# Ray0089/geometric-aware-dense-matching

Measured on AMD Instinct MI355X. Metric: rgbd_crops_per_sec_geomatch_fwd, higher is better.
Workload: dtype bf16x3/f32acc

## Files before the change

geometric_aware_dense_matching_amd/csrc/gdm_lfa.hip:

```cpp
#include "gdm_common.h"
#include <math.h>
#include <stdlib.h>

namespace {

constexpr int LK = 16;

struct LfaArgs {
    const float* xyz;
    const int32_t* idx;
    const float* feat;
    const float* w1t;
    const float* s1;
    const float* b1;
    const float* w2t;
    const float* s2;
    const float* b2;
    const float* wft;
    const float* wmt;
    const float* sm;
    const float* bm;
    float* out;
    int n, OUT;
    float slope;
};

__device__ __forceinline__ float lrelu(float v, float slope) { return v > 0.f ? v : v * slope; }



__device__ __forceinline__ float quadrow_max(float v)
{
    v = fmaxf(v, __shfl_xor(v, 16));
    v = fmaxf(v, __shfl_xor(v, 32));
    return v;
}
__device__ __forceinline__ float quadrow_sum(float v, int kq)
{
    float o = __shfl_xor(v, 16);
    v = (kq & 1) ? o + v : v + o;
    o = __shfl_xor(v, 32);
    v = (kq & 2) ? o + v : v + o;
    return v;
}

template <int ROWS, int KD, int NRT, int NPT, int WR, int WP>
__device__ __forceinline__ void lfa_tiles(const float* __restrict__ wt, const float* src, int src_pstride, int rt0, int pt0, int l16, int kq,
                                          gdm_f32x4 (&acc)[NRT][NPT])
{
#pragma unroll
    for (int i = 0; i < NRT; ++i)
#pragma unroll
        for (int j = 0; j < NPT; ++j)
#pragma unroll
            for (int r = 0; r < 4; ++r) acc[i][j][r] = 0.f;
    const float* wl = wt + (long)kq * ROWS + rt0 * 16 + l16;
    const float* sl = src + (long)pt0 * src_pstride + kq * LK + l16;
    constexpr int G = 4;
    static_assert(KD % (4 * G) == 0, "KD in whole groups");
    float an[G][NRT];
#pragma unroll
    for (int g = 0; g < G; ++g)
#pragma unroll
        for (int i = 0; i < NRT; ++i) an[g][i] = wl[(long)(4 * g) * ROWS + i * WR * 16];
    for (int jj = 0; jj < KD; jj += 4 * G) {
        float ac[G][NRT], bv[G][NPT];
#pragma unroll
        for (int g = 0; g < G; ++g)
#pragma unroll
            for (int i = 0; i < NRT; ++i) ac[g][i] = an[g][i];
        if (jj + 4 * G < KD) {
#pragma unroll
            for (int g = 0; g < G; ++g)
#pragma unroll
                for (int i = 0; i < NRT; ++i) an[g][i] = wl[(long)(jj + 4 * G + 4 * g) * ROWS + i * WR * 16];
        }
#pragma unroll
        for (int g = 0; g < G; ++g)
#pragma unroll
            for (int j = 0; j < NPT; ++j) bv[g][j] = sl[(jj + 4 * g) * LK + j * WP * src_pstride];
#pragma unroll
        for (int g = 0; g < G; ++g)
#pragma unroll
            for (int i = 0; i < NRT; ++i)
#pragma unroll
                for (int j = 0; j < NPT; ++j) acc[i][j] = __builtin_amdgcn_mfma_f32_16x16x4f32(bv[g][j], ac[g][i], acc[i][j], 0, 0, 0);
    }
}

template <int D, int PP>
__global__ __launch_bounds__(256) void lfa_stage_mfma_kernel(const LfaArgs a)
{
    constexpr int H = D / 2;
    constexpr int P = (256 / D) * PP;
    __shared__ __attribute__((aligned(16))) float fcat[P][D][LK];
    __shared__ __attribute__((aligned(16))) float fx1[P][H][LK];
    __shared__ float pe[P][10][LK];
    __shared__ int nidx[P][LK];
    __shared__ float aggv[P][D];

    const int tid = threadIdx.x;
    const int slot = tid / D, c = tid - slot * D;
    const int lane = tid & 63, wave = tid >> 6, l16 = lane & 15, kq = lane >> 4;
    const int b = blockIdx.y;
    const int n = a.n;
    const float slope = a.slope;
    int pidx[PP];
    bool live[PP];
#pragma unroll
    for (int pp = 0; pp < PP; ++pp) {
        const int raw = (int)blockIdx.x * P + slot * PP + pp;
        live[pp] = raw < n;
        pidx[pp] = min(raw, n - 1);
    }

    if (c < LK) {
#pragma unroll
        for (int pp = 0; pp < PP; ++pp) {
            const int p = slot * PP + pp, i = pidx[pp];
            int jn = a.idx[((long)b * n + i) * LK + c];
            jn = min(max(jn, 0), n - 1);
            const float* pi = a.xyz + ((long)b * n + i) * 3;
            const float* pj = a.xyz + ((long)b * n + jn) * 3;
            const float ax = pi[0], ay = pi[1], az = pi[2];
            const float bx = pj[0], by = pj[1], bz = pj[2];
            const float rx = __fsub_rn(ax, bx), ry = __fsub_rn(ay, by), rz = __fsub_rn(az, bz);
            float s = __fmul_rn(rx, rx);
            s = __fadd_rn(s, __fmul_rn(ry, ry));
            s = __fadd_rn(s, __fmul_rn(rz, rz));
            pe[p][0][c] = __fsqrt_rn(s);
            pe[p][1][c] = rx; pe[p][2][c] = ry; pe[p][3][c] = rz;
            pe[p][4][c] = ax; pe[p][5][c] = ay; pe[p][6][c] = az;
            pe[p][7][c] = bx; pe[p][8][c] = by; pe[p][9][c] = bz;
            nidx[p][c] = jn;
        }
    }
    __syncthreads();

    {
        const int j = c % H, kb = (c / H) * 8;
        float w[10];
#pragma unroll
        for (int q = 0; q < 10; ++q) w[q] = a.w1t[q * H + j];
        const float sc = a.s1[j], sh = a.b1[j];
        const float* frow = a.feat + ((long)b * H + j) * n;
#pragma unroll
        for (int pp = 0; pp < PP; ++pp) {
            const int p = slot * PP + pp;
#pragma unroll
            for (int kk = 0; kk < 8; ++kk) {
                const int k = kb + kk;
                float v = 0.f;
#pragma unroll
                for (int q = 0; q < 10; ++q) v = fmaf(w[q], pe[p][q][k], v);
                v = lrelu(fmaf(v, sc, sh), slope);
                if (a.w2t) fx1[p][j][k] = v;
                else fcat[p][H + j][k] = v;
                fcat[p][j][k] = frow[nidx[p][k]];
            }
        }
    }
    __syncthreads();

    if (a.w2t) {
        constexpr int RT = H / 16, WR = RT < 4 ? RT : 4, WP = 4 / WR, NRT = RT / WR, NPT = P / WP;
        static_assert(RT >= 1 && NRT * WR == RT && NPT * WP == P, "mlp2 tiling");
        const int wr = wave % WR, wp = wave / WR;
        gdm_f32x4 acc[NRT][NPT];
        lfa_tiles<H, H, NRT, NPT, WR, WP>(a.w2t, &fx1[0][0][0], H * LK, wr, wp, l16, kq, acc);
#pragma unroll
        for (int i = 0; i < NRT; ++i) {
            const int ch = (wr + WR * i) * 16 + l16;
            const float sc = a.s2[ch], sh = a.b2[ch];
#pragma unroll
            for (int j = 0; j < NPT; ++j) {
                float4 o;
                o.x = lrelu(fmaf(acc[i][j][0], sc, sh), slope); o.y = lrelu(fmaf(acc[i][j][1], sc, sh), slope);
                o.z = lrelu(fmaf(acc[i][j][2], sc, sh), slope); o.w = lrelu(fmaf(acc[i][j][3], sc, sh), slope);
                *reinterpret_cast<float4*>(&fcat[wp + WP * j][H + ch][4 * kq]) = o;
            }
        }
        __syncthreads();
    }

    {
        constexpr int RT = D / 16, WR = RT < 4 ? RT : 4, WP = 4 / WR, NRT = RT / WR, NPT = P / WP;
        static_assert(NRT * WR == RT && NPT * WP == P, "attention tiling");
        const int wr = wave % WR, wp = wave / WR;
        gdm_f32x4 acc[NRT][NPT];
        lfa_tiles<D, D, NRT, NPT, WR, WP>(a.wft, &fcat[0][0][0], D * LK, wr, wp, l16, kq, acc);
#pragma unroll
        for (int i = 0; i < NRT; ++i) {
            const int ch = (wr + WR * i) * 16 + l16;
#pragma unroll
            for (int j = 0; j < NPT; ++j) {
                const int p = wp + WP * j;
                const gdm_f32x4 t = acc[i][j];
                const float mx = quadrow_max(fmaxf(fmaxf(t[0], t[1]), fmaxf(t[2], t[3])));
                const float e0 = __expf(t[0] - mx), e1 = __expf(t[1] - mx), e2 = __expf(t[2] - mx), e3 = __expf(t[3] - mx);
                const float den = quadrow_sum((e0 + e1) + (e2 + e3), kq);
                const float4 f = *reinterpret_cast<const float4*>(&fcat[p][ch][4 * kq]);
                const float rden = 1.0f / den;
                const float num = quadrow_sum((f.x * (e0 * rden) + f.y * (e1 * rden)) + (f.z * (e2 * rden) + f.w * (e3 * rden)), kq);
                if (kq == 0) aggv[p][ch] = num;
            }
        }
    }
    __syncthreads();

    const int OUT = a.OUT;
    if (c < OUT) {
        float o[PP];
#pragma unroll
        for (int pp = 0; pp < PP; ++pp) o[pp] = 0.f;
#pragma unroll 8
        for (int jj = 0; jj < D; ++jj) {
            const float w = a.wmt[jj * OUT + c];
#pragma unroll
            for (int pp = 0; pp < PP; ++pp) o[pp] = fmaf(w, aggv[slot * PP + pp][jj], o[pp]);
        }
        const float sm = a.sm[c], bm = a.bm[c];
#pragma unroll
        for (int pp = 0; pp < PP; ++pp)
            if (live[pp]) a.out[((long)b * OUT + c) * n + pidx[pp]] = lrelu(fmaf(o[pp], sm, bm), slope);
    }
}

}

extern "C" int gdm_lfa_stage_hip(const float* xyz, const int32_t* idx, const float* feat, const float* w1t, const float* s1, const float* b1,
                                 const float* w2t, const float* s2, const float* b2, const float* wft, const float* wmt, const float* sm,
                                 const float* bm, int B, int n, int K, int D, int OUT, float slope, float* out, void* stream)
{
    GDM_CHECK_ARG(xyz && idx && feat && w1t && s1 && b1 && wft && wmt && sm && bm && out, "gdm_lfa_stage_hip: NULL pointer");
    GDM_CHECK_ARG(!w2t || (s2 && b2), "gdm_lfa_stage_hip: w2t without s2/b2");
    GDM_CHECK_ARG(K == LK, "gdm_lfa_stage_hip: K=%d, only K=16 is built", K);
    GDM_CHECK_ARG(D == 32 || D == 64 || D == 128 || D == 256, "gdm_lfa_stage_hip: D=%d not in {32,64,128,256}", D);
    GDM_CHECK_ARG(OUT >= 1 && OUT <= D, "gdm_lfa_stage_hip: OUT=%d must be in [1, D=%d]", OUT, D);
    GDM_CHECK_ARG(B >= 1 && B <= 65535 && n >= 1, "gdm_lfa_stage_hip: bad shape");
    LfaArgs a{xyz, idx, feat, w1t, s1, b1, w2t, s2, b2, wft, wmt, sm, bm, out, n, OUT, slope};
    hipStream_t s = (hipStream_t)stream;
    const int pp = D <= 64 ? 1 : 2;
    const int P = (256 / D) * pp;
    dim3 g(gdm_cdiv(n, P), B);
    if (D == 32) hipLaunchKernelGGL((lfa_stage_mfma_kernel<32, 1>), g, dim3(256), 0, s, a);
    else if (D == 64) hipLaunchKernelGGL((lfa_stage_mfma_kernel<64, 1>), g, dim3(256), 0, s, a);
    else if (D == 128) hipLaunchKernelGGL((lfa_stage_mfma_kernel<128, 2>), g, dim3(256), 0, s, a);
    else hipLaunchKernelGGL((lfa_stage_mfma_kernel<256, 2>), g, dim3(256), 0, s, a);
    return gdm_launch_status("lfa_stage_mfma_kernel");
}
```

geometric_aware_dense_matching_amd/csrc/gdm_pointwise.hip:

```cpp
#include "gdm_common.h"
#include <stdlib.h>

namespace {

constexpr int PT = 64, XS = 68;
constexpr int MAXSEG = 4;

struct PwSegDev {
    const float* x;
    const int32_t* idx;
    int C, n_src;
};

struct PwArgs {
    PwSegDev seg[MAXSEG];
    int nseg;
    const float* wt;
    long wks, wcs;
    const float* scale;
    const float* shift;
    float* out;
    int n, Cout, outC, out_c0, point_major, act, K;
    float slope;
    long total;
};

__device__ __forceinline__ const float* seg_column(const float* x, const int32_t* idx, int C, int n_src, long b, int i, long g)
{
    int col = i;
    if (idx) col = min(max(idx[g], 0), n_src - 1);
    return x + b * (long)C * n_src + col;
}

template <int NW, int KS, bool VEC>
__global__ __launch_bounds__(NW * 64) void pointwise_kernel(const PwArgs a)
{
    constexpr int NCG = NW / KS;
    constexpr int KT = 16;
    constexpr int XL = KT / NCG;
    constexpr int WL = KT / 4;
    static_assert(NCG >= 1 && NCG <= KT && KT % NCG == 0, "tile arrangement");
    __shared__ __attribute__((aligned(16))) float xs[KS][KT][XS];
    __shared__ __attribute__((aligned(16))) float ws[NW][KT][16];
    __shared__ __attribute__((aligned(16))) float red[KS > 1 ? NW : 1][16][64];
    const int tid = threadIdx.x;
    const int wave = tid >> 6, lane = tid & 63;
    const int cg = wave / KS, kp = wave % KS;
    const int tx = lane & 15, ty = lane >> 4;
    const long g0 = (long)blockIdx.x * PT;
    const int c0 = ((int)blockIdx.y * NCG + cg) * 16;
    const int n = a.n, Cout = a.Cout, K = a.K;
    const int kpart = (((K + KS - 1) / KS + KT - 1) / KT) * KT;
    const int kbeg = kp * kpart;
    const int nchunk = kpart / KT;

    const float *xb0, *xb1, *xb2;
    long xs0, xs1, xs2;
    int ce0, ce1;
    {
        const long g = min(g0 + (VEC ? (lane & 15) * 4 : lane), a.total - (VEC ? 4 : 1));
        const long b = g / n;
        const int i = (int)(g - b * n);
        xb0 = seg_column(a.seg[0].x, a.seg[0].idx, a.seg[0].C, a.seg[0].n_src, b, i, g);
        xs0 = a.seg[0].n_src;
        xb1 = xb2 = xb0;
        xs1 = xs2 = xs0;
        ce0 = a.seg[0].C;
        ce1 = ce0;
        if (a.nseg > 1) {
            xb1 = seg_column(a.seg[1].x, a.seg[1].idx, a.seg[1].C, a.seg[1].n_src, b, i, g);
            xs1 = a.seg[1].n_src;
            ce1 = ce0 + a.seg[1].C;
        }
        if (a.nseg > 2) {
            xb2 = seg_column(a.seg[2].x, a.seg[2].idx, a.seg[2].C, a.seg[2].n_src, b, i, g);
            xs2 = a.seg[2].n_src;
        }
    }
    const float* const wtp = a.wt;
    const long e1 = (const char*)xb1 - (const char*)xb0, e2 = (const char*)xb2 - (const char*)xb1;
    const long sd1 = xs1 - xs0, sd2 = xs2 - xs1;
    const int cd1 = ce0, cd2 = ce1 - ce0;
    auto x_addr = [&](int k) -> const float* {
        const int kc = min(k, K - 1);
        const long t1 = -(long)(kc >= ce0), t2 = -(long)(kc >= ce1);
        const int kl = kc - (cd1 & (int)t1) - (cd2 & (int)t2);
        const long str = xs0 + (sd1 & t1) + (sd2 & t2);
        const float* base = (const float*)((const char*)xb0 + (e1 & t1) + (e2 & t2));
        return base + (long)kl * str;
    };
    constexpr int XV = VEC ? XL / 4 : XL;
    constexpr int WV = VEC ? KT / 16 : WL;
    static_assert(!VEC || (XL % 4 == 0 && KT % 16 == 0), "vector loads cover 4 x rows / 16 w rows per instruction");
    const int wc = VEC ? min(c0 + (lane & 3) * 4, Cout - 4) : min(c0 + (lane & 15), Cout - 1);
    auto x_row = [&](int r) -> int { return VEC ? cg * XL + 4 * r + (lane >> 4) : cg + NCG * r; };
    auto w_row = [&](int r) -> int { return VEC ? 16 * r + (lane >> 2) : (lane >> 4) + 4 * r; };

    float acc[4][4];
#pragma unroll
    for (int j = 0; j < 4; ++j)
#pragma unroll
        for (int q = 0; q < 4; ++q) acc[j][q] = 0.f;

    float4 xr[XV], wr[WV];
    auto fetch = [&](int k0) {
#pragma unroll
        for (int r = 0; r < XV; ++r) {
            const float* p = x_addr(k0 + x_row(r));
            if (VEC) xr[r] = *reinterpret_cast<const float4*>(p);
            else xr[r].x = *p;
        }
#pragma unroll
        for (int r = 0; r < WV; ++r) {
            const float* p = wtp + (long)min(k0 + w_row(r), K - 1) * a.wks + (long)wc * a.wcs;
            if (VEC) wr[r] = *reinterpret_cast<const float4*>(p);
            else wr[r].x = *p;
        }
    };
    fetch(kbeg);
    for (int ch = 0; ch < nchunk; ++ch) {
        const int kc0 = kbeg + ch * KT;
#pragma unroll
        for (int r = 0; r < XV; ++r) {
            const bool in = kc0 + x_row(r) < K;
            if (VEC) *reinterpret_cast<float4*>(&xs[kp][x_row(r)][(lane & 15) * 4]) = in ? xr[r] : make_float4(0.f, 0.f, 0.f, 0.f);
            else xs[kp][x_row(r)][lane] = in ? xr[r].x : 0.f;
        }
#pragma unroll
        for (int r = 0; r < WV; ++r) {
            const bool in = kc0 + w_row(r) < K;
            if (VEC) *reinterpret_cast<float4*>(&ws[wave][w_row(r)][(lane & 3) * 4]) = in ? wr[r] : make_float4(0.f, 0.f, 0.f, 0.f);
            else ws[wave][w_row(r)][lane & 15] = in ? wr[r].x : 0.f;
        }
        __syncthreads();
        if (ch + 1 < nchunk) fetch(kbeg + (ch + 1) * KT);
        float4 xv[2][4], wv[2][4];
#pragma unroll
        for (int u = 0; u < 4; ++u) {
            xv[0][u] = *reinterpret_cast<const float4*>(&xs[kp][u][tx * 4]);
            wv[0][u] = *reinterpret_cast<const float4*>(&ws[wave][u][ty * 4]);
        }
#pragma unroll
        for (int k4 = 0; k4 < KT / 4; ++k4) {
            const int cur = k4 & 1, nxt = cur ^ 1;
            if (k4 + 1 < KT / 4) {
#pragma unroll
                for (int u = 0; u < 4; ++u) {
                    xv[nxt][u] = *reinterpret_cast<const float4*>(&xs[kp][(k4 + 1) * 4 + u][tx * 4]);
                    wv[nxt][u] = *reinterpret_cast<const float4*>(&ws[wave][(k4 + 1) * 4 + u][ty * 4]);
                }
            }
#pragma unroll
            for (int u = 0; u < 4; ++u) {
                const float4 x4 = xv[cur][u], w4 = wv[cur][u];
                acc[0][0] = fmaf(w4.x, x4.x, acc[0][0]); acc[0][1] = fmaf(w4.x, x4.y, acc[0][1]);
                acc[0][2] = fmaf(w4.x, x4.z, acc[0][2]); acc[0][3] = fmaf(w4.x, x4.w, acc[0][3]);
                acc[1][0] = fmaf(w4.y, x4.x, acc[1][0]); acc[1][1] = fmaf(w4.y, x4.y, acc[1][1]);
                acc[1][2] = fmaf(w4.y, x4.z, acc[1][2]); acc[1][3] = fmaf(w4.y, x4.w, acc[1][3]);
                acc[2][0] = fmaf(w4.z, x4.x, acc[2][0]); acc[2][1] = fmaf(w4.z, x4.y, acc[2][1]);
                acc[2][2] = fmaf(w4.z, x4.z, acc[2][2]); acc[2][3] = fmaf(w4.z, x4.w, acc[2][3]);
                acc[3][0] = fmaf(w4.w, x4.x, acc[3][0]); acc[3][1] = fmaf(w4.w, x4.y, acc[3][1]);
                acc[3][2] = fmaf(w4.w, x4.z, acc[3][2]); acc[3][3] = fmaf(w4.w, x4.w, acc[3][3]);
            }
        }
        __syncthreads();
    }
    if (KS > 1) {
        if (kp != 0) {
#pragma unroll
            for (int j = 0; j < 4; ++j)
#pragma unroll
                for (int q = 0; q < 4; ++q) red[wave][j * 4 + q][lane] = acc[j][q];
        }
        __syncthreads();
        if (kp != 0) return;
        for (int p = 1; p < KS; ++p)
#pragma unroll
            for (int j = 0; j < 4; ++j)
#pragma unroll
                for (int q = 0; q < 4; ++q) acc[j][q] += red[cg * KS + p][j * 4 + q][lane];
    }

    const long p0 = g0 + tx * 4;
    float v[4][4];
#pragma unroll
    for (int j = 0; j < 4; ++j) {
        const int c = c0 + ty * 4 + j;
        const bool live = c < Cout;
        const float sc = (live && a.scale) ? a.scale[c] : 1.f;
        const float sh = (live && a.shift) ? a.shift[c] : 0.f;
#pragma unroll
        for (int q = 0; q < 4; ++q) {
            float y = fmaf(acc[j][q], sc, sh);
            if (a.act == 1) y = fmaxf(y, 0.f);
            else if (a.act == 2) y = y > 0.f ? y : y * a.slope;
            v[j][q] = y;
        }
    }
    if (a.point_major) {
        const int c = c0 + ty * 4;
        const bool vec = (a.outC % 4 == 0) && (a.out_c0 % 4 == 0) && (c + 3 < Cout);
#pragma unroll
        for (int q = 0; q < 4; ++q) {
            const long p = p0 + q;
            if (p >= a.total) continue;
            float* o = a.out + p * a.outC + a.out_c0 + c;
            if (vec) *reinterpret_cast<float4*>(o) = make_float4(v[0][q], v[1][q], v[2][q], v[3][q]);
            else
                for (int j = 0; j < 4; ++j)
                    if (c + j < Cout) o[j] = v[j][q];
        }
    } else {
        const bool vec = (n % 4 == 0) && (p0 + 3 < a.total);
        const long b = p0 < a.total ? p0 / n : 0;
        const int i = (int)(p0 - b * n);
#pragma unroll
        for (int j = 0; j < 4; ++j) {
            const int c = c0 + ty * 4 + j;
            if (c >= Cout) continue;
            if (vec) {
                float* o = a.out + ((long)b * a.outC + a.out_c0 + c) * n + i;
                *reinterpret_cast<float4*>(o) = make_float4(v[j][0], v[j][1], v[j][2], v[j][3]);
            } else {
                for (int q = 0; q < 4; ++q) {
                    const long p = p0 + q;
                    if (p >= a.total) break;
                    const long bb = p / n;
                    a.out[((long)bb * a.outC + a.out_c0 + c) * n + (p - bb * n)] = v[j][q];
                }
            }
        }
    }
}


template <int KS, bool VEC, int CB = 1>
__device__ __forceinline__ void pw_mfma_tile(const PwArgs& a, const long p0, const int c0, float (*red)[16][64])
{
    static_assert(CB == 1 || KS == 1, "several channel blocks per wave only without a K split");
    const int tid = threadIdx.x, wave = KS > 1 ? tid >> 6 : 0, lane = tid & 63;
    const int l16 = lane & 15, kq = lane >> 4;
    const int n = a.n, Cout = a.Cout, K = a.K;
    const int kpart = (((K + KS - 1) / KS + 3) / 4) * 4;
    const int kbeg = wave * kpart, kend = min(K, kbeg + kpart);

    long pb[4];
    int pi[4];
    long pg[4];
#pragma unroll
    for (int g = 0; g < 4; ++g) {
        const long p = VEC ? min(p0 + 4 * l16, a.total - 4) + g : min(p0 + 16 * g + l16, a.total - 1);
        pg[g] = p;
        pb[g] = p / n;
        pi[g] = (int)(p - pb[g] * n);
    }
    long wcoff[CB];
#pragma unroll
    for (int cb = 0; cb < CB; ++cb) wcoff[cb] = (long)min(c0 + 16 * cb + l16, Cout - 1) * a.wcs;

    gdm_f32x4 acc[CB][4];
#pragma unroll
    for (int cb = 0; cb < CB; ++cb)
#pragma unroll
        for (int g = 0; g < 4; ++g)
#pragma unroll
            for (int r = 0; r < 4; ++r) acc[cb][g][r] = 0.f;

    int seg_start = 0;
#pragma unroll
    for (int s = 0; s < MAXSEG; ++s) {
        if (s >= a.nseg) break;
        const float* sx = a.seg[s].x;
        const int32_t* sidx = a.seg[s].idx;
        const int sC = a.seg[s].C, sn = a.seg[s].n_src;
        const int seg_end = seg_start + sC;
        const int k0 = max(kbeg, seg_start), k1 = min(kend, seg_end);
        if (k0 < k1) {
            const float* xp[4];
#pragma unroll
            for (int g = 0; g < 4; ++g) {
                int col = pi[g];
                if (sidx) col = min(max(sidx[pg[g]], 0), sn - 1);
                xp[g] = sx + (pb[g] * sC + (k0 - seg_start + kq)) * (long)sn + col;
            }
            const float* wp = a.wt + (long)(k0 + kq) * a.wks;
            const long xinc = 4L * sn, winc = 4L * a.wks;
            const int nfull = (k1 - k0) / 4;
            const int ngrp = nfull / 4;
            float xa[4][4], wa[4][CB], xb[4][4], wb[4][CB];
            auto load_grp = [&](float (&xv)[4][4], float (&wv)[4][CB]) {
#pragma unroll
                for (int u = 0; u < 4; ++u) {
#pragma unroll
                    for (int cb = 0; cb < CB; ++cb) wv[u][cb] = wp[wcoff[cb]];
                    wp += winc;
                    if (VEC) {
                        const float4 t = *reinterpret_cast<const float4*>(xp[0]);
                        xv[u][0] = t.x; xv[u][1] = t.y; xv[u][2] = t.z; xv[u][3] = t.w;
                        xp[0] += xinc;
                    } else {
#pragma unroll
                        for (int g = 0; g < 4; ++g) {
                            xv[u][g] = xp[g][0];
                            xp[g] += xinc;
                        }
                    }
                }
            };
            auto mfma_grp = [&](const float (&xv)[4][4], const float (&wv)[4][CB]) {
#pragma unroll
                for (int u = 0; u < 4; ++u)
#pragma unroll
                    for (int cb = 0; cb < CB; ++cb)
#pragma unroll
                        for (int g = 0; g < 4; ++g) acc[cb][g] = __builtin_amdgcn_mfma_f32_16x16x4f32(xv[u][g], wv[u][cb], acc[cb][g], 0, 0, 0);
            };
            int st = 4 * ngrp;
            if (ngrp > 0) {
                load_grp(xa, wa);
                int gi = 0;
                for (; gi + 2 < ngrp; gi += 2) {
                    load_grp(xb, wb);
                    mfma_grp(xa, wa);
                    load_grp(xa, wa);
                    mfma_grp(xb, wb);
                }
                if (gi + 1 < ngrp) {
                    load_grp(xb, wb);
                    mfma_grp(xa, wa);
                    mfma_grp(xb, wb);
                } else {
                    mfma_grp(xa, wa);
                }
            }
            for (; st < nfull; ++st) {
                float wv[CB];
#pragma unroll
                for (int cb = 0; cb < CB; ++cb) wv[cb] = wp[wcoff[cb]];
                wp += winc;
                float xv[4];
                if (VEC) {
                    const float4 t = *reinterpret_cast<const float4*>(xp[0]);
                    xv[0] = t.x; xv[1] = t.y; xv[2] = t.z; xv[3] = t.w;
                    xp[0] += xinc;
                } else {
#pragma unroll
                    for (int g = 0; g < 4; ++g) {
                        xv[g] = xp[g][0];
                        xp[g] += xinc;
                    }
                }
#pragma unroll
                for (int cb = 0; cb < CB; ++cb)
#pragma unroll
                    for (int g = 0; g < 4; ++g) acc[cb][g] = __builtin_amdgcn_mfma_f32_16x16x4f32(xv[g], wv[cb], acc[cb][g], 0, 0, 0);
            }
            if (k0 + 4 * nfull < k1) {
                const bool in = k0 + 4 * nfull + kq < k1;
                const long back = in ? 0 : (long)(k0 + 4 * nfull + kq - (k1 - 1));
                float wv[CB];
#pragma unroll
                for (int cb = 0; cb < CB; ++cb) {
                    const float wraw = wp[wcoff[cb] - back * a.wks];
                    wv[cb] = in ? wraw : 0.f;
                }
                float xraw[4];
                if (VEC) {
                    const float4 t = *reinterpret_cast<const float4*>(xp[0] - back * sn);
                    xraw[0] = t.x; xraw[1] = t.y; xraw[2] = t.z; xraw[3] = t.w;
                } else {
#pragma unroll
                    for (int g = 0; g < 4; ++g) xraw[g] = xp[g][-back * sn];
                }
#pragma unroll
                for (int cb = 0; cb < CB; ++cb)
#pragma unroll
                    for (int g = 0; g < 4; ++g) acc[cb][g] = __builtin_amdgcn_mfma_f32_16x16x4f32(in ? xraw[g] : 0.f, wv[cb], acc[cb][g], 0, 0, 0);
            }
        }
        seg_start = seg_end;
    }

    if (KS > 1) {
        if (wave != 0) {
#pragma unroll
            for (int g = 0; g < 4; ++g)
#pragma unroll
                for (int r = 0; r < 4; ++r) red[wave][g * 4 + r][lane] = acc[0][g][r];
        }
        __syncthreads();
        if (wave != 0) return;
        for (int w = 1; w < KS; ++w)
#pragma unroll
            for (int g = 0; g < 4; ++g)
#pragma unroll
                for (int r = 0; r < 4; ++r) acc[0][g][r] += red[w][g * 4 + r][lane];
    }

#pragma unroll
    for (int cb = 0; cb < CB; ++cb) {
    const int co = c0 + 16 * cb + l16;
    if (co >= Cout) continue;
    const float sc = a.scale ? a.scale[co] : 1.f, sh = a.shift ? a.shift[co] : 0.f;
    auto finish = [&](float y) {
        y = fmaf(y, sc, sh);
        if (a.act == 1) y = fmaxf(y, 0.f);
        else if (a.act == 2) y = y > 0.f ? y : y * a.slope;
        return y;
    };
#pragma unroll
    for (int j = 0; j < 4; ++j) {
        float v[4];
#pragma unroll
        for (int i = 0; i < 4; ++i) v[i] = finish(VEC ? acc[cb][i][j] : acc[cb][j][i]);
        const long q0 = p0 + (VEC ? 16 * kq + 4 * j : 16 * j + 4 * kq);
        if (a.point_major) {
#pragma unroll
            for (int r = 0; r < 4; ++r)
                if (q0 + r < a.total) a.out[(q0 + r) * a.outC + a.out_c0 + co] = v[r];
        } else if (n % 4 == 0 && q0 + 3 < a.total) {
            const long b = q0 / n;
            *reinterpret_cast<float4*>(a.out + (b * a.outC + a.out_c0 + co) * n + (q0 - b * n)) = make_float4(v[0], v[1], v[2], v[3]);
        } else {
#pragma unroll
            for (int r = 0; r < 4; ++r) {
                const long q = q0 + r;
                if (q >= a.total) break;
                const long b = q / n;
                a.out[(b * a.outC + a.out_c0 + co) * n + (q - b * n)] = v[r];
            }
        }
    }
    }
}

template <int KS, bool VEC, int CB = 1>
__global__ __launch_bounds__(KS * 64) void pointwise_mfma_kernel(const PwArgs a)
{
    __shared__ __attribute__((aligned(16))) float red[KS > 1 ? KS : 1][16][64];
    pw_mfma_tile<KS, VEC, CB>(a, (long)blockIdx.x * PT, (int)blockIdx.y * (16 * CB), red);
}

template <bool VEC, int CB>
__global__ __launch_bounds__(256) void pointwise_mfma_cw_kernel(const PwArgs a)
{
    const int wave = __builtin_amdgcn_readfirstlane((int)threadIdx.x >> 6);
    const int c0 = ((int)blockIdx.y * 4 + wave) * (16 * CB);
    if (c0 >= a.Cout) return;
    pw_mfma_tile<1, VEC, CB>(a, (long)blockIdx.x * PT, c0, nullptr);
}

template <int KS>
__global__ __launch_bounds__(KS * 64) void pointwise_mfma_jobs_kernel(const PwArgs a0, const PwArgs a1, const PwArgs a2, const PwArgs a3,
                                                                      int e0, int e1, int e2, int vecmask)
{
    __shared__ __attribute__((aligned(16))) float red[KS > 1 ? KS : 1][16][64];
    const int bx = (int)blockIdx.x, c0 = (int)blockIdx.y * 16;
    if (bx < e0) {
        if (vecmask & 1) pw_mfma_tile<KS, true>(a0, (long)bx * PT, c0, red);
        else pw_mfma_tile<KS, false>(a0, (long)bx * PT, c0, red);
    } else if (bx < e1) {
        if (vecmask & 2) pw_mfma_tile<KS, true>(a1, (long)(bx - e0) * PT, c0, red);
        else pw_mfma_tile<KS, false>(a1, (long)(bx - e0) * PT, c0, red);
    } else if (bx < e2) {
        if (vecmask & 4) pw_mfma_tile<KS, true>(a2, (long)(bx - e1) * PT, c0, red);
        else pw_mfma_tile<KS, false>(a2, (long)(bx - e1) * PT, c0, red);
    } else {
        if (vecmask & 8) pw_mfma_tile<KS, true>(a3, (long)(bx - e2) * PT, c0, red);
        else pw_mfma_tile<KS, false>(a3, (long)(bx - e2) * PT, c0, red);
    }
}

struct PwChain2 {
    const float* x;
    const float *w0t, *s0, *b0;
    const float *w1t, *s1, *b1;
    float *y0, *y1;
    int n, C0, C1, C2, act0, act1;
    float slope0, slope1;
    long total;
};

__device__ __forceinline__ float pw_act(float y, int act, float slope)
{
    if (act == 1) return fmaxf(y, 0.f);
    if (act == 2) return y > 0.f ? y : y * slope;
    return y;
}

__global__ __launch_bounds__(256) void pointwise_chain2_kernel(const PwChain2 a)
{
    constexpr int CMAX0 = 16, CMAX1 = 16, CMAX2 = 32;
    const long g = (long)blockIdx.x * 256 + threadIdx.x;
    if (g >= a.total) return;
    const long b = g / a.n;
    const int i = (int)(g - b * a.n);
    float xin[CMAX0];
#pragma unroll
    for (int k = 0; k < CMAX0; ++k) xin[k] = k < a.C0 ? a.x[(b * a.C0 + k) * a.n + i] : 0.f;
    float h[CMAX1];
#pragma unroll
    for (int c = 0; c < CMAX1; ++c) {
        float acc = 0.f;
        if (c < a.C1) {
#pragma unroll
            for (int k = 0; k < CMAX0; ++k)
                if (k < a.C0) acc = fmaf(a.w0t[k * a.C1 + c], xin[k], acc);
            acc = pw_act(fmaf(acc, a.s0 ? a.s0[c] : 1.f, a.b0 ? a.b0[c] : 0.f), a.act0, a.slope0);
            a.y0[(b * a.C1 + c) * a.n + i] = acc;
        }
        h[c] = acc;
    }
#pragma unroll
    for (int c = 0; c < CMAX2; ++c) {
        if (c < a.C2) {
            float acc = 0.f;
#pragma unroll
            for (int k = 0; k < CMAX1; ++k)
                if (k < a.C1) acc = fmaf(a.w1t[k * a.C2 + c], h[k], acc);
            a.y1[(b * a.C2 + c) * a.n + i] = pw_act(fmaf(acc, a.s1 ? a.s1[c] : 1.f, a.b1 ? a.b1[c] : 0.f), a.act1, a.slope1);
        }
    }
}

bool seg_ok(const gdm_pw_seg& s, int n)
{
    return s.x && s.C >= 1 && s.n_src >= 1 && (s.idx || s.n_src == n);
}

}

extern "C" int gdm_pointwise2_hip(const gdm_pw_seg* segs, int nseg, const float* wt, int w_rowmajor, const float* scale, const float* shift,
                                  int B, int n, int Cout, int act, float slope, float* out, int out_C, int out_c0, int point_major,
                                  void* stream)
{
    GDM_CHECK_ARG(segs && wt && out, "gdm_pointwise2_hip: NULL pointer");
    GDM_CHECK_ARG(nseg >= 1 && nseg <= MAXSEG, "gdm_pointwise2_hip: nseg=%d not in [1,%d]", nseg, MAXSEG);
    GDM_CHECK_ARG(B >= 1 && n >= 1 && Cout >= 1, "gdm_pointwise2_hip: bad shape B=%d n=%d Cout=%d", B, n, Cout);
    GDM_CHECK_ARG(out_c0 >= 0 && out_c0 + Cout <= out_C, "gdm_pointwise2_hip: channels [%d, %d) outside the output's %d", out_c0,
                  out_c0 + Cout, out_C);
    GDM_CHECK_ARG(act >= 0 && act <= 2, "gdm_pointwise2_hip: act=%d", act);
    PwArgs a;
    a.K = 0;
    for (int s = 0; s < MAXSEG; ++s) {
        if (s < nseg) {
            GDM_CHECK_ARG(seg_ok(segs[s], n), "gdm_pointwise2_hip: segment %d: NULL / empty, or n_src=%d != n=%d without an index", s,
                          segs[s].n_src, n);
            a.seg[s] = PwSegDev{segs[s].x, segs[s].idx, segs[s].C, segs[s].n_src};
            a.K += segs[s].C;
        } else
            a.seg[s] = PwSegDev{nullptr, nullptr, 0, 0};
    }
    GDM_CHECK_ARG(((uintptr_t)out & 15) == 0, "gdm_pointwise2_hip: out must be 16-byte aligned");
    a.nseg = nseg;
    a.wt = wt;
    a.wks = w_rowmajor ? 1 : Cout;
    a.wcs = w_rowmajor ? a.K : 1;
    a.scale = scale;
    a.shift = shift;
    a.out = out;
    a.n = n;
    a.Cout = Cout;
    a.outC = out_C;
    a.out_c0 = out_c0;
    a.point_major = point_major ? 1 : 0;
    a.act = act;
    a.slope = slope;
    a.total = (long)B * n;
    const long tiles = (a.total + PT - 1) / PT;
    GDM_CHECK_ARG(tiles <= 0x7fffffffL, "gdm_pointwise2_hip: grid too large");
    hipStream_t st = (hipStream_t)stream;
    bool vec = (n % 4 == 0) && (Cout % 4 == 0) && (((uintptr_t)wt & 15) == 0) && !w_rowmajor;
    for (int s = 0; s < nseg; ++s) vec = vec && !segs[s].idx && (((uintptr_t)segs[s].x & 15) == 0);
    if (a.K >= 32 && gdm_cdiv(Cout, 16) <= 65535) {
        int ks = 1;
        while (ks < 8 && a.K / (2 * ks) >= 16 && tiles * gdm_cdiv(Cout, 16) * ks < 4096) ks *= 2;
        const dim3 grid((unsigned)tiles, gdm_cdiv(Cout, 16));
        bool mvec = (n % 4 == 0);
        for (int sgi = 0; sgi < nseg; ++sgi) mvec = mvec && !segs[sgi].idx && (((uintptr_t)segs[sgi].x & 15) == 0) && segs[sgi].n_src % 4 == 0;
        if (ks == 1 && Cout >= 32 && tiles >= 1024) {
            const dim3 gridc((unsigned)tiles, gdm_cdiv(Cout, 64));
            if (mvec) hipLaunchKernelGGL((pointwise_mfma_cw_kernel<true, 1>), gridc, dim3(256), 0, st, a);
            else hipLaunchKernelGGL((pointwise_mfma_cw_kernel<false, 1>), gridc, dim3(256), 0, st, a);
            return gdm_launch_status("pointwise_mfma_cw_kernel");
        }
        gdm_dispatch_int<4>(__builtin_ctz(ks), [&](auto L) {
            constexpr int KSV = 1 << decltype(L)::value;
            gdm_dispatch_bool(mvec, [&](auto V) {
                hipLaunchKernelGGL((pointwise_mfma_kernel<KSV, decltype(V)::value>), grid, dim3(KSV * 64), 0, st, a);
            });
        });
        return gdm_launch_status("pointwise_mfma_kernel");
    }
    GDM_CHECK_ARG(nseg <= 3, "gdm_pointwise2_hip: four segments need K >= 32 (the MFMA form)");
    const dim3 grid((unsigned)tiles, gdm_cdiv(Cout, 64));
    if (vec) hipLaunchKernelGGL((pointwise_kernel<4, 1, true>), grid, dim3(256), 0, st, a);
    else hipLaunchKernelGGL((pointwise_kernel<4, 1, false>), grid, dim3(256), 0, st, a);
    return gdm_launch_status("pointwise_kernel");
}

extern "C" int gdm_pointwise_jobs_hip(const gdm_pw_job* jobs, int njobs, int B, int K, int Cout, void* stream)
{
    GDM_CHECK_ARG(jobs && njobs >= 1 && njobs <= 4, "gdm_pointwise_jobs_hip: njobs=%d not in [1,4]", njobs);
    GDM_CHECK_ARG(B >= 1 && K >= 32 && Cout >= 1 && gdm_cdiv(Cout, 16) <= 65535, "gdm_pointwise_jobs_hip: bad shape B=%d K=%d Cout=%d", B, K, Cout);
    int kjob[4] = {0, 0, 0, 0};
    for (int j = 0; j < njobs; ++j) {
        const gdm_pw_job& jb = jobs[j];
        GDM_CHECK_ARG(jb.x && jb.wt && jb.out && jb.n >= 1, "gdm_pointwise_jobs_hip: job %d: NULL pointer or n=%d", j, jb.n);
        GDM_CHECK_ARG(((uintptr_t)jb.out & 15) == 0, "gdm_pointwise_jobs_hip: job %d: out must be 16-byte aligned", j);
        const long tj = ((long)B * jb.n + PT - 1) / PT;
        int kj = 1;
        while (kj < 8 && K / (2 * kj) >= 16 && tj * gdm_cdiv(Cout, 16) * kj < 4096) kj *= 2;
        kjob[j] = kj;
    }
    hipStream_t st = (hipStream_t)stream;
    for (int ks = 1; ks <= 8; ks *= 2) {
        PwArgs a[4];
        int ends[4];
        int vecmask = 0, m = 0;
        long tiles = 0;
        const gdm_pw_job* last = nullptr;
        for (int j = 0; j < njobs; ++j) {
            if (kjob[j] != ks) continue;
            const gdm_pw_job& jb = jobs[j];
            last = &jb;
            for (int sgi = 0; sgi < MAXSEG; ++sgi) a[m].seg[sgi] = PwSegDev{nullptr, nullptr, 0, 0};
            a[m].seg[0] = PwSegDev{jb.x, nullptr, K, jb.n};
            a[m].nseg = 1;
            a[m].wt = jb.wt;
            a[m].wks = Cout;
            a[m].wcs = 1;
            a[m].scale = nullptr;
            a[m].shift = nullptr;
            a[m].out = jb.out;
            a[m].n = jb.n;
            a[m].Cout = Cout;
            a[m].outC = Cout;
            a[m].out_c0 = 0;
            a[m].point_major = 0;
            a[m].act = 0;
            a[m].slope = 0.f;
            a[m].K = K;
            a[m].total = (long)B * jb.n;
            tiles += (a[m].total + PT - 1) / PT;
            if (jb.n % 4 == 0 && ((uintptr_t)jb.x & 15) == 0) vecmask |= 1 << m;
            ends[m] = (int)tiles;
            ++m;
        }
        if (m == 0) continue;
        for (int q = m; q < 4; ++q) {
            a[q] = a[m - 1];
            ends[q] = (int)tiles;
        }
        (void)last;
        GDM_CHECK_ARG(tiles <= 0x7fffffffL, "gdm_pointwise_jobs_hip: grid too large");
        const dim3 grid((unsigned)tiles, gdm_cdiv(Cout, 16));
        gdm_dispatch_int<4>(__builtin_ctz(ks), [&](auto L) {
            constexpr int KSV = 1 << decltype(L)::value;
            hipLaunchKernelGGL((pointwise_mfma_jobs_kernel<KSV>), grid, dim3(KSV * 64), 0, st, a[0], a[1], a[2], a[3], ends[0], ends[1], ends[2], vecmask);
        });
        const int rc = gdm_launch_status("pointwise_mfma_jobs_kernel");
        if (rc) return rc;
    }
    return 0;
}

extern "C" int gdm_pointwise_chain2_hip(const float* x, const float* w0t, const float* s0, const float* b0, int act0, float slope0,
                                        const float* w1t, const float* s1, const float* b1, int act1, float slope1,
                                        int B, int n, int C0, int C1, int C2, float* y0, float* y1, void* stream)
{
    GDM_CHECK_ARG(x && w0t && w1t && y0 && y1, "gdm_pointwise_chain2_hip: NULL pointer");
    GDM_CHECK_ARG(B >= 1 && n >= 1 && C0 >= 1 && C0 <= 16 && C1 >= 1 && C1 <= 16 && C2 >= 1 && C2 <= 32,
                  "gdm_pointwise_chain2_hip: B=%d n=%d C0=%d (<= 16) C1=%d (<= 16) C2=%d (<= 32)", B, n, C0, C1, C2);
    GDM_CHECK_ARG(act0 >= 0 && act0 <= 2 && act1 >= 0 && act1 <= 2, "gdm_pointwise_chain2_hip: act=%d,%d", act0, act1);
    PwChain2 a;
    a.x = x; a.w0t = w0t; a.s0 = s0; a.b0 = b0; a.w1t = w1t; a.s1 = s1; a.b1 = b1; a.y0 = y0; a.y1 = y1;
    a.n = n; a.C0 = C0; a.C1 = C1; a.C2 = C2; a.act0 = act0; a.act1 = act1; a.slope0 = slope0; a.slope1 = slope1;
    a.total = (long)B * n;
    GDM_CHECK_ARG(gdm_cdiv(a.total, 256) <= 0x7fffffff, "gdm_pointwise_chain2_hip: grid too large");
    hipLaunchKernelGGL(pointwise_chain2_kernel, dim3(gdm_cdiv(a.total, 256)), dim3(256), 0, (hipStream_t)stream, a);
    return gdm_launch_status("pointwise_chain2_kernel");
}
```

Measured before the change: 5384.

## Hoist LFA global loads ahead of syncs and add fixed-shape pointwise chain kernel

The LFA stage kernel now issues its neighbour indices, own xyz, gathered features, MLP weights, scales and the first MFMA weight groups for both matmuls before the first barrier, so their latency overlaps the geometry stage. The weight prefetch in the MFMA tile loop becomes two groups deep, and an occupancy hint (waves per EU) is added. The shared-memory neighbour index buffer is dropped. Separately, a templated chain2 kernel for the 9->8->16 shape spreads the output channels across four waves per 64 points. The cost is higher register pressure and duplicated first-layer compute across waves.

Result: no change. 5395 (median of 5 runs) (+0.2%).

```diff
diff --git a/geometric_aware_dense_matching_amd/csrc/gdm_lfa.hip b/geometric_aware_dense_matching_amd/csrc/gdm_lfa.hip
--- a/geometric_aware_dense_matching_amd/csrc/gdm_lfa.hip
+++ b/geometric_aware_dense_matching_amd/csrc/gdm_lfa.hip
@@ -44,9 +44,23 @@
     return v;
 }
 
-template <int ROWS, int KD, int NRT, int NPT, int WR, int WP>
+constexpr int LG = 4;
+
+template <int NPF, int ROWS, int KD, int NRT, int WR>
+__device__ __forceinline__ void lfa_w_first(const float* __restrict__ wt, int rt0, int l16, int kq, float (&an)[NPF][LG][NRT])
+{
+    const float* wl = wt + (long)kq * ROWS + rt0 * 16 + l16;
+#pragma unroll
+    for (int d = 0; d < NPF; ++d)
+#pragma unroll
+        for (int g = 0; g < LG; ++g)
+#pragma unroll
+            for (int i = 0; i < NRT; ++i) an[d][g][i] = d * 4 * LG < KD ? wl[(long)(d * 4 * LG + 4 * g) * ROWS + i * WR * 16] : 0.f;
+}
+
+template <int NPF, int ROWS, int KD, int NRT, int NPT, int WR, int WP>
 __device__ __forceinline__ void lfa_tiles(const float* __restrict__ wt, const float* src, int src_pstride, int rt0, int pt0, int l16, int kq,
-                                          gdm_f32x4 (&acc)[NRT][NPT])
+                                          float (&an)[NPF][LG][NRT], gdm_f32x4 (&acc)[NRT][NPT])
 {
 #pragma unroll
     for (int i = 0; i < NRT; ++i)
@@ -56,48 +70,51 @@
             for (int r = 0; r < 4; ++r) acc[i][j][r] = 0.f;
     const float* wl = wt + (long)kq * ROWS + rt0 * 16 + l16;
     const float* sl = src + (long)pt0 * src_pstride + kq * LK + l16;
-    constexpr int G = 4;
-    static_assert(KD % (4 * G) == 0, "KD in whole groups");
-    float an[G][NRT];
-#pragma unroll
-    for (int g = 0; g < G; ++g)
-#pragma unroll
-        for (int i = 0; i < NRT; ++i) an[g][i] = wl[(long)(4 * g) * ROWS + i * WR * 16];
-    for (int jj = 0; jj < KD; jj += 4 * G) {
-        float ac[G][NRT], bv[G][NPT];
-#pragma unroll
-        for (int g = 0; g < G; ++g)
-#pragma unroll
-            for (int i = 0; i < NRT; ++i) ac[g][i] = an[g][i];
-        if (jj + 4 * G < KD) {
-#pragma unroll
-            for (int g = 0; g < G; ++g)
-#pragma unroll
-                for (int i = 0; i < NRT; ++i) an[g][i] = wl[(long)(jj + 4 * G + 4 * g) * ROWS + i * WR * 16];
-        }
-#pragma unroll
-        for (int g = 0; g < G; ++g)
-#pragma unroll
-            for (int j = 0; j < NPT; ++j) bv[g][j] = sl[(jj + 4 * g) * LK + j * WP * src_pstride];
-#pragma unroll
-        for (int g = 0; g < G; ++g)
-#pragma unroll
-            for (int i = 0; i < NRT; ++i)
-#pragma unroll
-                for (int j = 0; j < NPT; ++j) acc[i][j] = __builtin_amdgcn_mfma_f32_16x16x4f32(bv[g][j], ac[g][i], acc[i][j], 0, 0, 0);
+    static_assert(KD % (4 * LG) == 0, "KD in whole groups");
+    for (int jb = 0; jb < KD; jb += NPF * 4 * LG) {
+#pragma unroll
+        for (int d = 0; d < NPF; ++d) {
+            const int jj = jb + d * 4 * LG;
+            if (KD % (NPF * 4 * LG) != 0 && jj >= KD) break;
+            float ac[LG][NRT], bv[LG][NPT];
+#pragma unroll
+            for (int g = 0; g < LG; ++g)
+#pragma unroll
+                for (int i = 0; i < NRT; ++i) ac[g][i] = an[d][g][i];
+            if (jj + NPF * 4 * LG < KD) {
+#pragma unroll
+                for (int g = 0; g < LG; ++g)
+#pragma unroll
+                    for (int i = 0; i < NRT; ++i) an[d][g][i] = wl[(long)(jj + NPF * 4 * LG + 4 * g) * ROWS + i * WR * 16];
+            }
+#pragma unroll
+            for (int g = 0; g < LG; ++g)
+#pragma unroll
+                for (int j = 0; j < NPT; ++j) bv[g][j] = sl[(jj + 4 * g) * LK + j * WP * src_pstride];
+#pragma unroll
+            for (int g = 0; g < LG; ++g)
+#pragma unroll
+                for (int i = 0; i < NRT; ++i)
+#pragma unroll
+                    for (int j = 0; j < NPT; ++j) acc[i][j] = __builtin_amdgcn_mfma_f32_16x16x4f32(bv[g][j], ac[g][i], acc[i][j], 0, 0, 0);
+        }
     }
 }
 
 template <int D, int PP>
-__global__ __launch_bounds__(256) void lfa_stage_mfma_kernel(const LfaArgs a)
+__global__ __launch_bounds__(256) __attribute__((amdgpu_waves_per_eu(D <= 64 ? 5 : 3))) void lfa_stage_mfma_kernel(const LfaArgs a)
 {
     constexpr int H = D / 2;
     constexpr int P = (256 / D) * PP;
+    constexpr int NPF = 2;
     __shared__ __attribute__((aligned(16))) float fcat[P][D][LK];
     __shared__ __attribute__((aligned(16))) float fx1[P][H][LK];
     __shared__ float pe[P][10][LK];
-    __shared__ int nidx[P][LK];
     __shared__ float aggv[P][D];
+    constexpr int RT2 = H / 16, WR2 = RT2 < 4 ? RT2 : 4, WP2 = 4 / WR2, NRT2 = RT2 / WR2, NPT2 = P / WP2;
+    constexpr int RT3 = D / 16, WR3 = RT3 < 4 ? RT3 : 4, WP3 = 4 / WR3, NRT3 = RT3 / WR3, NPT3 = P / WP3;
+    static_assert(RT2 >= 1 && NRT2 * WR2 == RT2 && NPT2 * WP2 == P, "mlp2 tiling");
+    static_assert(NRT3 * WR3 == RT3 && NPT3 * WP3 == P, "attention tiling");
 
     const int tid = threadIdx.x;
     const int slot = tid / D, c = tid - slot * D;
@@ -114,15 +131,57 @@
         pidx[pp] = min(raw, n - 1);
     }
 
+    const int j1 = c % H, kb = (c / H) * 8;
+    const int wr2 = wave % WR2, wp2 = wave / WR2, wr3 = wave % WR3, wp3 = wave / WR3;
+    const bool second = a.w2t != nullptr;
+    int jn[PP];
+    float own[PP][3];
+#pragma unroll
+    for (int pp = 0; pp < PP; ++pp) {
+        jn[pp] = a.idx[((long)b * n + pidx[pp]) * LK + (c & (LK - 1))];
+        const float* pi = a.xyz + ((long)b * n + pidx[pp]) * 3;
+        own[pp][0] = pi[0]; own[pp][1] = pi[1]; own[pp][2] = pi[2];
+    }
+    int gi[PP][8];
+#pragma unroll
+    for (int pp = 0; pp < PP; ++pp)
+#pragma unroll
+        for (int kk = 0; kk < 8; ++kk) gi[pp][kk] = a.idx[((long)b * n + pidx[pp]) * LK + kb + kk];
+    float w1[10];
+#pragma unroll
+    for (int q = 0; q < 10; ++q) w1[q] = a.w1t[q * H + j1];
+    const float sc1 = a.s1[j1], sh1 = a.b1[j1];
+    float an2[NPF][LG][NRT2], s2v[NRT2], b2v[NRT2];
+    lfa_w_first<NPF, H, H, NRT2, WR2>(second ? a.w2t : a.wft, wr2, l16, kq, an2);
+    {
+        const float *s2p = second ? a.s2 : a.s1, *b2p = second ? a.b2 : a.b1;
+#pragma unroll
+        for (int i = 0; i < NRT2; ++i) {
+            s2v[i] = s2p[(wr2 + WR2 * i) * 16 + l16];
+            b2v[i] = b2p[(wr2 + WR2 * i) * 16 + l16];
+        }
+    }
+    float an3[NPF][LG][NRT3];
+    lfa_w_first<NPF, D, D, NRT3, WR3>(a.wft, wr3, l16, kq, an3);
+    const int OUT = a.OUT;
+    const float smv = a.sm[min(c, OUT - 1)], bmv = a.bm[min(c, OUT - 1)];
+    float fv[PP][8];
+    {
+        const float* frow = a.feat + ((long)b * H + j1) * n;
+#pragma unroll
+        for (int pp = 0; pp < PP; ++pp)
+#pragma unroll
+            for (int kk = 0; kk < 8; ++kk) fv[pp][kk] = frow[min(max(gi[pp][kk], 0), n - 1)];
+    }
+#pragma unroll
+    for (int pp = 0; pp < PP; ++pp) asm volatile("" : "+v"(jn[pp]), "+v"(own[pp][0]), "+v"(own[pp][1]), "+v"(own[pp][2]));
+
     if (c < LK) {
 #pragma unroll
         for (int pp = 0; pp < PP; ++pp) {
-            const int p = slot * PP + pp, i = pidx[pp];
-            int jn = a.idx[((long)b * n + i) * LK + c];
-            jn = min(max(jn, 0), n - 1);
-            const float* pi = a.xyz + ((long)b * n + i) * 3;
-            const float* pj = a.xyz + ((long)b * n + jn) * 3;
-            const float ax = pi[0], ay = pi[1], az = pi[2];
+            const int p = slot * PP + pp;
+            const float* pj = a.xyz + ((long)b * n + min(max(jn[pp], 0), n - 1)) * 3;
+            const float ax = own[pp][0], ay = own[pp][1], az = own[pp][2];
             const float bx = pj[0], by = pj[1], bz = pj[2];
             const float rx = __fsub_rn(ax, bx), ry = __fsub_rn(ay, by), rz = __fsub_rn(az, bz);
             float s = __fmul_rn(rx, rx);
@@ -132,18 +191,12 @@
             pe[p][1][c] = rx; pe[p][2][c] = ry; pe[p][3][c] = rz;
             pe[p][4][c] = ax; pe[p][5][c] = ay; pe[p][6][c] = az;
             pe[p][7][c] = bx; pe[p][8][c] = by; pe[p][9][c] = bz;
-            nidx[p][c] = jn;
         }
     }
     __syncthreads();
 
     {
-        const int j = c % H, kb = (c / H) * 8;
-        float w[10];
-#pragma unroll
-        for (int q = 0; q < 10; ++q) w[q] = a.w1t[q * H + j];
-        const float sc = a.s1[j], sh = a.b1[j];
-        const float* frow = a.feat + ((long)b * H + j) * n;
+        const int j = j1;
 #pragma unroll
         for (int pp = 0; pp < PP; ++pp) {
             const int p = slot * PP + pp;
@@ -152,26 +205,25 @@
                 const int k = kb + kk;
                 float v = 0.f;
 #pragma unroll
-                for (int q = 0; q < 10; ++q) v = fmaf(w[q], pe[p][q][k], v);
-                v = lrelu(fmaf(v, sc, sh), slope);
-                if (a.w2t) fx1[p][j][k] = v;
+                for (int q = 0; q < 10; ++q) v = fmaf(w1[q], pe[p][q][k], v);
+                v = lrelu(fmaf(v, sc1, sh1), slope);
+                if (second) fx1[p][j][k] = v;
                 else fcat[p][H + j][k] = v;
-                fcat[p][j][k] = frow[nidx[p][k]];
+                fcat[p][j][k] = fv[pp][kk];
             }
         }
     }
     __syncthreads();
 
-    if (a.w2t) {
-        constexpr int RT = H / 16, WR = RT < 4 ? RT : 4, WP = 4 / WR, NRT = RT / WR, NPT = P / WP;
-        static_assert(RT >= 1 && NRT * WR == RT && NPT * WP == P, "mlp2 tiling");
-        const int wr = wave % WR, wp = wave / WR;
+    if (second) {
+        constexpr int WR = WR2, WP = WP2, NRT = NRT2, NPT = NPT2;
+        const int wr = wr2, wp = wp2;
         gdm_f32x4 acc[NRT][NPT];
-        lfa_tiles<H, H, NRT, NPT, WR, WP>(a.w2t, &fx1[0][0][0], H * LK, wr, wp, l16, kq, acc);
+        lfa_tiles<NPF, H, H, NRT, NPT, WR, WP>(a.w2t, &fx1[0][0][0], H * LK, wr, wp, l16, kq, an2, acc);
 #pragma unroll
         for (int i = 0; i < NRT; ++i) {
             const int ch = (wr + WR * i) * 16 + l16;
-            const float sc = a.s2[ch], sh = a.b2[ch];
+            const float sc = s2v[i], sh = b2v[i];
 #pragma unroll
             for (int j = 0; j < NPT; ++j) {
                 float4 o;
@@ -184,11 +236,10 @@
     }
 
     {
-        constexpr int RT = D / 16, WR = RT < 4 ? RT : 4, WP = 4 / WR, NRT = RT / WR, NPT = P / WP;
-        static_assert(NRT * WR == RT && NPT * WP == P, "attention tiling");
-        const int wr = wave % WR, wp = wave / WR;
+        constexpr int WR = WR3, WP = WP3, NRT = NRT3, NPT = NPT3;
+        const int wr = wr3, wp = wp3;
         gdm_f32x4 acc[NRT][NPT];
-        lfa_tiles<D, D, NRT, NPT, WR, WP>(a.wft, &fcat[0][0][0], D * LK, wr, wp, l16, kq, acc);
+        lfa_tiles<NPF, D, D, NRT, NPT, WR, WP>(a.wft, &fcat[0][0][0], D * LK, wr, wp, l16, kq, an3, acc);
 #pragma unroll
         for (int i = 0; i < NRT; ++i) {
             const int ch = (wr + WR * i) * 16 + l16;
@@ -208,7 +259,6 @@
     }
     __syncthreads();
 
-    const int OUT = a.OUT;
     if (c < OUT) {
         float o[PP];
 #pragma unroll
@@ -219,10 +269,9 @@
 #pragma unroll
             for (int pp = 0; pp < PP; ++pp) o[pp] = fmaf(w, aggv[slot * PP + pp][jj], o[pp]);
         }
-        const float sm = a.sm[c], bm = a.bm[c];
 #pragma unroll
         for (int pp = 0; pp < PP; ++pp)
-            if (live[pp]) a.out[((long)b * OUT + c) * n + pidx[pp]] = lrelu(fmaf(o[pp], sm, bm), slope);
+            if (live[pp]) a.out[((long)b * OUT + c) * n + pidx[pp]] = lrelu(fmaf(o[pp], smv, bmv), slope);
     }
 }
 
diff --git a/geometric_aware_dense_matching_amd/csrc/gdm_pointwise.hip b/geometric_aware_dense_matching_amd/csrc/gdm_pointwise.hip
--- a/geometric_aware_dense_matching_amd/csrc/gdm_pointwise.hip
+++ b/geometric_aware_dense_matching_amd/csrc/gdm_pointwise.hip
@@ -520,6 +520,39 @@
                 if (k < a.C1) acc = fmaf(a.w1t[k * a.C2 + c], h[k], acc);
             a.y1[(b * a.C2 + c) * a.n + i] = pw_act(fmaf(acc, a.s1 ? a.s1[c] : 1.f, a.b1 ? a.b1[c] : 0.f), a.act1, a.slope1);
         }
+    }
+}
+
+template <int C0, int C1, int C2, int GR>
+__global__ __launch_bounds__(64 * GR) void pointwise_chain2_fixed_kernel(const PwChain2 a)
+{
+    static_assert(C1 % GR == 0 && C2 % GR == 0, "whole channel groups");
+    const int g = __builtin_amdgcn_readfirstlane((int)threadIdx.x >> 6);
+    const long pt = (long)blockIdx.x * 64 + (threadIdx.x & 63);
+    if (pt >= a.total) return;
+    const long b = pt / a.n;
+    const int i = (int)(pt - b * a.n);
+    float xin[C0];
+#pragma unroll
+    for (int k = 0; k < C0; ++k) xin[k] = a.x[(b * C0 + k) * a.n + i];
+    float h[C1];
+#pragma unroll
+    for (int c = 0; c < C1; ++c) {
+        float acc = 0.f;
+#pragma unroll
+        for (int k = 0; k < C0; ++k) acc = fmaf(a.w0t[k * C1 + c], xin[k], acc);
+        h[c] = pw_act(fmaf(acc, a.s0 ? a.s0[c] : 1.f, a.b0 ? a.b0[c] : 0.f), a.act0, a.slope0);
+    }
+#pragma unroll
+    for (int c = 0; c < C1; ++c)
+        if (c / (C1 / GR) == g) a.y0[(b * C1 + c) * a.n + i] = h[c];
+#pragma unroll
+    for (int cc = 0; cc < C2 / GR; ++cc) {
+        const int c = g * (C2 / GR) + cc;
+        float acc = 0.f;
+#pragma unroll
+        for (int k = 0; k < C1; ++k) acc = fmaf(a.w1t[k * C2 + c], h[k], acc);
+        a.y1[(b * C2 + c) * a.n + i] = pw_act(fmaf(acc, a.s1 ? a.s1[c] : 1.f, a.b1 ? a.b1[c] : 0.f), a.act1, a.slope1);
     }
 }
 
@@ -677,7 +710,11 @@
     a.x = x; a.w0t = w0t; a.s0 = s0; a.b0 = b0; a.w1t = w1t; a.s1 = s1; a.b1 = b1; a.y0 = y0; a.y1 = y1;
     a.n = n; a.C0 = C0; a.C1 = C1; a.C2 = C2; a.act0 = act0; a.act1 = act1; a.slope0 = slope0; a.slope1 = slope1;
     a.total = (long)B * n;
-    GDM_CHECK_ARG(gdm_cdiv(a.total, 256) <= 0x7fffffff, "gdm_pointwise_chain2_hip: grid too large");
+    GDM_CHECK_ARG(gdm_cdiv(a.total, 64) <= 0x7fffffff, "gdm_pointwise_chain2_hip: grid too large");
+    if (C0 == 9 && C1 == 8 && C2 == 16) {
+        hipLaunchKernelGGL((pointwise_chain2_fixed_kernel<9, 8, 16, 4>), dim3(gdm_cdiv(a.total, 64)), dim3(256), 0, (hipStream_t)stream, a);
+        return gdm_launch_status("pointwise_chain2_fixed_kernel");
+    }
     hipLaunchKernelGGL(pointwise_chain2_kernel, dim3(gdm_cdiv(a.total, 256)), dim3(256), 0, (hipStream_t)stream, a);
     return gdm_launch_status("pointwise_chain2_kernel");
 }
```
